# tenstack/batch-scheduler

Hardware: AMD Instinct MI355X
Metric: pod x node fit evals/sec (higher is better)
Workload: dtype int64; 1 GPU; cfg3/tail: 10000 pods / 2000 groups / 5000 nodes, 5 int64 lanes (cpu, mem, eph, pods, gpu), seed 20260921; stages=prefilter+filter+tally+ready, parallelism=single GPU

## Files before the change

### batch-scheduler_amd/csrc/bs_fast.hpp

```cpp
#pragma once

#include "bs_kernels.hpp"
#include "bs_filter_t.hpp"

#ifdef BS_NT_TABLES
#define BS_TBL_STORE(p, v) __builtin_nontemporal_store((v), (p))
#else
#define BS_TBL_STORE(p, v) (*(p) = (v))
#endif
namespace bs {

template <bool INL = false>
__device__ __forceinline__ void arm_tally(const GroupsDev& gr, const BatchDev& b, const BatchParams& prm, uint32_t i, uint32_t nthreads);

__device__ __forceinline__ const uint8_t* range_glocal(const BatchDev& b) { return reinterpret_cast<const uint8_t*>(b.pod_ranges); }
__device__ __forceinline__ const uint32_t* range_start(const BatchDev& b, uint32_t G) { return b.pod_ranges + (G + 3u) / 4u; }
__device__ __forceinline__ const uint32_t* range_lfirst(const BatchDev& b, uint32_t G, uint32_t pod_blocks) { return range_start(b, G) + pod_blocks + 1u; }
__device__ __forceinline__ bool range_local_on(const BatchDev& b, const BatchParams& prm) {
  return b.pod_ranges && prm.do_tally && prm.do_ready && !prm.filter_deny;
}

#if BS_EMIT_MAIN
__global__ void k_pods_prep(unsigned long long* tables, uint32_t ntab, uint32_t* gstat, uint32_t ngstat, uint32_t* kcount, uint32_t* gcount, uint32_t G) {
  const uint32_t t = blockIdx.x * blockDim.x + threadIdx.x, nt = gridDim.x * blockDim.x;
// ... 166 lines not shown
      al[j] = nd.alloc[(size_t)j * nd.stride + n];
      rq[j] = nd.req[(size_t)j * nd.stride + n];
    }
  }
  const bool fit = valid && ((fw >> (n & 31u)) & 1u) && !(fl & BS_NODE_TAINT_ERR);
  const uint32_t pres = fit ? (ap & rp) : 0u;
  BS_STAMP(1, 1);
  if (threadIdx.x < BS_MAX_SCALARS) s_kp[threadIdx.x] = BS_INF;
  unsigned long long incl[BS_MAX_LANES];
  const int w = wave_id();
#pragma unroll
  for (uint32_t j = 0; j < BS_MAX_LANES; ++j) {
    if (j < L) {
      const bool live = fit && (j < 4 || (pres & (1u << (j - 4)))) && !(j == BS_LANE_EPH && !prm.eph_gate);
      const unsigned long long left = live ? (unsigned long long)wsub(scale_f32(al[j], d.pct), rq[j]) : 0ull;
      incl[j] = wave_incl_scan_add_u64(left);
      if (lane_id() == 63) s_wtot[j][w] = incl[j];
    }
  }
  __syncthreads();
#pragma unroll
  for (uint32_t j = 0; j < BS_MAX_LANES; ++j) {
    if (j < L) {
      unsigned long long off = 0, tot = 0;
#pragma unroll
      for (int i = 0; i < 4; ++i) {
        const unsigned long long x = s_wtot[j][i];
        if (i < w) off += x;
        tot += x;
      }
      incl[j] += off;
      if (valid) BS_TBL_STORE(&T[(size_t)k * LP + j], (int64_t)incl[j]);
      if (threadIdx.x == 0) b.chunk_tot[(size_t)chunk * 16 + j] = tot;
    } else if (j < LP && valid) {
      BS_TBL_STORE(&T[(size_t)k * LP + j], (int64_t)INT64_MAX);
    }
  }
  {
    const uint32_t grp = k >> 6;
    const bool grp_valid = (chunk * kTblChunk + (threadIdx.x & ~63u)) < nd.m;
    constexpr int64_t kSafe = (int64_t)1 << 62;
#pragma unroll
    for (uint32_t j = 0; j < BS_MAX_LANES; ++j) {
      if (j < L) {
        const int64_t x = (int64_t)incl[j];
        const long long mx = wave_max_i64_lane63(valid ? x : INT64_MIN);
        const bool risky = __ballot(valid && (x >= kSafe || x <= -kSafe)) != 0ull;
        if (lane_id() == 63 && grp_valid) b.gmax[(size_t)grp * LP + j] = risky ? INT64_MAX : mx;
      }
    }
  }
#pragma unroll
  for (uint32_t s = 0; s < BS_MAX_SCALARS; ++s) {
    if (s < S) {
      const unsigned long long mk = __ballot(valid && (pres & (1u << s)));
      if (mk && lane_id() == 0) atomicMin(&s_kp[s], chunk * kTblChunk + (uint32_t)(threadIdx.x & ~63u) + (uint32_t)(__ffsll((long long)mk) - 1));
    }
  }
  __syncthreads();
  if (threadIdx.x < 16) b.chunk_kp[(size_t)chunk * 16 + threadIdx.x] = threadIdx.x < BS_MAX_SCALARS ? s_kp[threadIdx.x] : BS_INF;
}

struct LeaderPre { Res mr; bool have_mr; int64_t min_member, status_scheduled, matched; };
template <bool PUB, typename T>
__device__ __forceinline__ void st_pub(T* p, T v) {
  if constexpr (PUB) __hip_atomic_store(p, v, __ATOMIC_RELAXED, __HIP_MEMORY_SCOPE_AGENT);
  else *p = v;
}
#ifndef BS_HOME_WT
#define BS_HOME_WT 0
#endif
template <typename T>
__device__ __forceinline__ void st_home(T* p, T v) {
#if BS_HOME_WT
  __hip_atomic_store(p, v, __ATOMIC_RELAXED, __HIP_MEMORY_SCOPE_SYSTEM);
#else
  *p = v;
#endif
}
__device__ __forceinline__ uint32_t ld_agent(const uint32_t* p) { return __hip_atomic_load(p, __ATOMIC_RELAXED, __HIP_MEMORY_SCOPE_AGENT); }
__device__ __forceinline__ unsigned long long ld_agent64(const void* p) {
  return __hip_atomic_load(reinterpret_cast<const unsigned long long*>(p), __ATOMIC_RELAXED, __HIP_MEMORY_SCOPE_AGENT);
}
template <int TS>
__device__ __forceinline__ void leader_pre_load(const GroupsDev& gr, int32_t leader, Shape<TS> sh, LeaderPre& o) {
  const uint32_t l = leader >= 0 ? (uint32_t)leader : 0u;
#pragma unroll
  for (uint32_t j = 0; j < BS_MAX_LANES; ++j) o.mr.v[j] = j < sh.L() ? gr.minres[(size_t)j * gr.g + l] : 0;
  o.mr.present = gr.mrpres[l];
  o.have_mr = (gr.flags[l] & BS_GROUP_HAS_MINRES) != 0;
  o.min_member = (int64_t)gr.min_member[l];
  o.status_scheduled = (int64_t)gr.status_scheduled[l];
  o.matched = (int64_t)gr.matched[l];
}
template <int TS>
__device__ __forceinline__ void pre_allocated_from(const LeaderPre& lp, Shape<TS> sh, uint32_t gate, Res& out) {
  res_zero(out, sh);
  const int64_t mm = lp.min_member;
  const int64_t not_finished = lp.matched != 0 ? mm - lp.matched : mm - lp.status_scheduled;
  if (not_finished > 0 && lp.have_mr) {
    Res times;
#pragma unroll
    for (uint32_t j = 0; j < BS_MAX_LANES; ++j)
      if (j < sh.L()) times.v[j] = wmul(lp.mr.v[j], not_finished);
    times.present = lp.mr.present;
    res_add(out, times, sh, gate);
  }
  if (out.v[BS_LANE_PODS] == 0) out.v[BS_LANE_PODS] = mm + 1;
}
template <int TS>
__device__ __forceinline__ uint32_t filter_slot_values(const Res& cur_in, const LeaderPre& lp, Shape<TS> sh, uint32_t gate, int64_t (&R)[4], int64_t (&M)[4]) {
  Res ms, cur = cur_in;
  res_zero(ms, sh);
  res_add(ms, lp.mr, sh, gate);
  res_add(cur, ms, sh, gate);
  uint32_t ff = 0;
#pragma unroll
  for (uint32_t s = 0; s < BS_MAX_SCALARS; ++s) {
    if (s < sh.S()) {
      if ((cur.present & (1u << s)) && cur.v[4 + s] != 0) ff |= 1u;
      if ((ms.present & (1u << s)) && ms.v[4 + s] != 0) ff |= 2u;
    }
  }
#pragma unroll
  for (int j = 0; j < 4; ++j) { R[j] = cur.v[j]; M[j] = ms.v[j]; }
  return ff;
}
template <int TS, bool PUB = false>
__device__ __forceinline__ void filter_slot_from(const BatchDev& b, const BatchParams& prm, const Res& cur_in, const LeaderPre& lp, Shape<TS> sh, uint32_t gate,
                                                 uint32_t slot, bool zero_feas = true) {
  if (!lp.have_mr) return;
  int64_t R[4], M[4];
  const uint32_t ff = filter_slot_values(cur_in, lp, sh, gate, R, M);
  if (zero_feas) st_pub<PUB>(&b.fu_feas[slot], 0u);
  int64_t* dst2 = b.uparams + (size_t)slot * 8;
#pragma unroll
  for (int j = 0; j < 4; ++j) { st_pub<PUB>(&dst2[j], R[j]); st_pub<PUB>(&dst2[4 + j], M[j]); }
  st_pub<PUB>(&b.uflags[slot], ff | ((uint32_t)BS_FL_EVALUATED << 8) | (prm.stamp << 16));
}
template <int TS>
__device__ __forceinline__ uint32_t class_scan_query(const Res& cur, const LeaderPre& lp0, Shape<TS> sh, uint32_t gate, Res& q) {
  pre_allocated_from(lp0, sh, gate, q);
  res_add(q, cur, sh, gate);
  uint32_t absok = 0;
#pragma unroll
  for (uint32_t s2 = 0; s2 < BS_MAX_SCALARS; ++s2) {
    if (s2 < sh.S()) {
      const bool pres = q.present & (1u << s2);
      if (!pres || q.v[4 + s2] == 0) absok |= 1u << s2;
      if (!pres) q.v[4 + s2] = INT64_MIN;
    }
  }
  return q.present | (absok << 16);
}

template <int TS, bool PUB = false, bool SLOTS = true, bool INL = false>
__device__ __forceinline__ void fast_query_thread(const PodsDev& pods, const GroupsDev& gr, const BatchDev& b, const BatchParams& prm, uint32_t i,
                                                  uint32_t nthreads, uint32_t end = BS_INF, uint32_t t = BS_INF) {
  const Shape<TS> sh(prm.S);
  const bool valid = i < pods.p && i < end;
  const uint32_t gate = prm.eph_gate;
  const uint32_t ii = valid ? i : 0u;
  const int32_t leader0 = b.leader_epoch[0];
  const uint8_t panic0 = b.panic_epoch[0];
  const uint32_t K = prm.run_filter ? (prm.k_host ? prm.k_host : *b.kclass) : 0u;
  const int32_t gi = pods.p ? pods.group[ii] : BS_POD_NOT_GROUPED;
  const uint8_t pfl = pods.p ? pods.flags[ii] : (uint8_t)0;
  const uint64_t own = pods.p ? pods.owner[ii] : 0ull;
  const uint32_t pc = pods.p ? b.pclass[ii] : 0u;
  const uint32_t pp = pods.p ? b.ppair[ii] : BS_INF;
  Res cur;
  if (pods.p) pod_require(pods, ii, sh, gate, cur); else res_zero(cur, sh);
  arm_tally<INL>(gr, b, prm, t == BS_INF ? i : t, nthreads);
  if (i < 8 && prm.collect_stats) b.stats[i] = 0;
  const bool grouped = valid && gi >= 0 && (uint32_t)gi < gr.g;
  const uint32_t g = grouped ? (uint32_t)gi : 0u;
// ... 152 lines not shown
template <int TS>
__global__ __launch_bounds__(kTblChunk) void k_fast_query_tables(PodsDev pods, GroupsDev gr, NodesDev nd, BatchDev b, BatchDev bt, BatchParams prm,
                                                                 const TableDesc* forced, uint32_t nchunks, uint32_t query_blocks) {
  BS_STAMP(1, 0);
  if (blockIdx.x < query_blocks) fast_query_thread<TS>(pods, gr, b, prm, blockIdx.x * kTblChunk + threadIdx.x, query_blocks * kTblChunk);
  else if (blockIdx.x < query_blocks + nchunks) tables_local_fast<TS>(nd, bt, prm, forced, blockIdx.x - query_blocks);
  else node_words_block<TS>(gr, nd, b, prm, blockIdx.x - query_blocks - nchunks);
  BS_STAMP(1, 7);
}

template <int NL>
__device__ __forceinline__ unsigned long long rows_cover(unsigned long long m, const int64_t (&a)[BS_MAX_LANES], const int64_t (&r)[BS_MAX_LANES]) {
  asm volatile("s_mov_b64 exec, %[m]\n\tv_cmpx_ge_i64 vcc, %[a0], %[r0]\n\tv_cmpx_ge_i64 vcc, %[a1], %[r1]\n\tv_cmpx_ge_i64 vcc, %[a2], %[r2]\n\t"
               "v_cmpx_ge_i64 vcc, %[a3], %[r3]\n\ts_mov_b64 %[m], exec\n\ts_mov_b64 exec, -1"
               : [m] "+s"(m)
               : [a0] "v"(a[0]), [r0] "v"(r[0]), [a1] "v"(a[1]), [r1] "v"(r[1]), [a2] "v"(a[2]), [r2] "v"(r[2]), [a3] "v"(a[3]), [r3] "v"(r[3])
               : "vcc");
#pragma unroll
  for (int j = 4; j < NL; ++j)
    asm volatile("s_mov_b64 exec, %[m]\n\tv_cmpx_ge_i64 vcc, %[a], %[r]\n\ts_mov_b64 %[m], exec\n\ts_mov_b64 exec, -1" : [m] "+s"(m) : [a] "v"(a[j]), [r] "v"(r[j]) : "vcc");
  return m;
}
#ifndef BS_SCAN_BALLOT
#define BS_SCAN_BALLOT 1
#endif
constexpr uint32_t kSpinBound = 1u << 18;
__device__ __forceinline__ void test_chaos_delay() {
#ifdef BS_TEST_CHAOS
  uint32_t h = (blockIdx.x + 1u) * 2654435761u ^ (uint32_t)wall_clock64() * 40503u;
  h ^= h >> 15; h *= 2246822519u; h ^= h >> 13;
  for (uint32_t s = 0; s < (h & 15u); ++s) __builtin_amdgcn_s_sleep(127);
#endif
}
constexpr uint32_t kStepSlotsMax = 256;
__device__ __forceinline__ bool step_wait(const uint32_t* word, uint32_t base, uint32_t need, int32_t* h_err) {
  uint32_t spins = 0;
  while ((uint32_t)(ld_agent(word) - base) < need) {
    __builtin_amdgcn_s_sleep(1);
    if (++spins > kSpinBound) { if (h_err) __hip_atomic_store(h_err, 1, __ATOMIC_RELAXED, __HIP_MEMORY_SCOPE_SYSTEM); return false; }
  }
  return true;
}
constexpr uint32_t kScanRecChunks = 64;
constexpr uint32_t kFeasRecGroups = 32;
#ifndef BS_GATHER_DIRECT
#define BS_GATHER_DIRECT 8
#endif
constexpr uint32_t kGatherDirectBlocks = BS_GATHER_DIRECT;
constexpr uint32_t kRecStride = 32;
constexpr uint32_t kTkSlots = 32, kTkTab = 48, kTkP1 = 64, kTkDone = 64 + 16 * 16, kTkWays = 16, kTkWords = 64 + 2 * 16 * 16;
__device__ __forceinline__ void spread_add(uint32_t* words, uint32_t who) {
  (void)__hip_atomic_fetch_add(&words[16u * (who % kTkWays)], 1u, __ATOMIC_RELAXED, __HIP_MEMORY_SCOPE_AGENT);
}
__device__ __forceinline__ bool spread_wait(const uint32_t* words, uint32_t base, uint32_t need, int32_t* h_err) {
  uint32_t spins = 0;
  for (;;) {
    uint32_t v = lane_id() < (int)kTkWays ? ld_agent(&words[16u * (uint32_t)lane_id()]) : 0u;
#pragma unroll
    for (int o = 1; o < (int)kTkWays; o <<= 1) v += (uint32_t)__shfl_xor((int)v, o);
    v = (uint32_t)__builtin_amdgcn_readfirstlane((int)v);
    if ((uint32_t)(v - base) >= need) return true;
    __builtin_amdgcn_s_sleep(4);
    if (++spins > kSpinBound) { if (h_err && lane_id() == 0) __hip_atomic_store(h_err, 1, __ATOMIC_RELAXED, __HIP_MEMORY_SCOPE_SYSTEM); return false; }
  }
}
template <int TS, bool REGS = false>
__device__ __forceinline__ void table_scan_block(const NodesDev& nd, const BatchDev& b, const BatchParams& prm, const TableDesc* forced, uint32_t chunk, uint32_t nchunks,
                                                 uint32_t share, uint32_t nshares, uint32_t pod_blocks, uint32_t tk_pods0, uint32_t tk_tab0, const GroupsDev& gr,
                                                 const int64_t* ckeys, const uint32_t* cpres, uint32_t kcap, bool direct = false, uint32_t forced_cls = 0) {
  __shared__ unsigned long long s_wtot[BS_MAX_LANES][4];
  __shared__ uint32_t s_kp[BS_MAX_SCALARS];
  __shared__ unsigned long long s_off[BS_MAX_LANES];
  __shared__ uint32_t s_kpg[BS_MAX_SCALARS];
  __shared__ int64_t s_req[kStepSlotsMax][BS_MAX_LANES];
  __shared__ uint32_t s_qf[kStepSlotsMax];
  __shared__ uint32_t s_first[kStepSlotsMax];
  BS_STAMP(2, 0);
  const Shape<TS> sh(prm.S);
  const uint32_t L = sh.L(), S = sh.S(), LP = prm.LP;
  const uint32_t k = chunk * kTblChunk + threadIdx.x;
  const bool in_range = REGS ? k < nd.n : k < nd.m;
  const uint32_t n = REGS ? (in_range ? k : 0u) : (in_range ? nd.kmap[k] : 0u);
  const TableDesc d = REGS ? TableDesc{forced_cls, 0.7f} : *forced;
  const uint32_t fw = nd.fit[(size_t)d.cls * nd.fit_words + (n >> 5)];
  const uint8_t fl = nd.flags[n];
  const bool valid = in_range && (!REGS || !(fl & BS_NODE_SKIP_MASK));
  const uint32_t ap = nd.apres[n], rp = nd.rpres[n];
  int64_t al[BS_MAX_LANES], rq[BS_MAX_LANES];
#pragma unroll
  for (uint32_t j = 0; j < BS_MAX_LANES; ++j) {
    if (j < L) {
      al[j] = nd.alloc[(size_t)j * nd.stride + n];
      rq[j] = nd.req[(size_t)j * nd.stride + n];
    }
  }
  const uint32_t K = prm.k_host ? prm.k_host : *b.kclass;
  const uint32_t per = (K + nshares - 1u) / nshares, s_lo = share * per, s_hi = min(K, s_lo + per);
  Res raw;
  int32_t leader0 = -1;
  uint8_t panic0 = 0;
  LeaderPre lp0{};
  if constexpr (REGS) {
    const uint32_t cc = s_lo + threadIdx.x < s_hi ? s_lo + threadIdx.x : 0u;
#pragma unroll
    for (uint32_t j = 0; j < BS_MAX_LANES; ++j)
      if (j < L) raw.v[j] = ckeys[(size_t)j * kcap + cc];
    raw.present = cpres[cc];
    leader0 = b.leader_epoch[0];
    panic0 = b.panic_epoch[0];
    if (gr.g) leader_pre_load(gr, leader0, sh, lp0);
  }
  const bool fit = valid && ((fw >> (n & 31u)) & 1u) && !(fl & BS_NODE_TAINT_ERR);
  const uint32_t pres = fit ? (ap & rp) : 0u;
  if (threadIdx.x < BS_MAX_SCALARS) s_kp[threadIdx.x] = BS_INF;
  for (uint32_t t = threadIdx.x; t < kStepSlotsMax; t += kTblChunk) s_first[t] = BS_INF;
  unsigned long long incl[BS_MAX_LANES];
  const int w = wave_id();
#pragma unroll
  for (uint32_t j = 0; j < BS_MAX_LANES; ++j) {
    incl[j] = 0;
    if (j < L) {
      const bool live = fit && (j < 4 || (pres & (1u << (j - 4)))) && !(j == BS_LANE_EPH && !prm.eph_gate);
      const unsigned long long left = live ? (unsigned long long)wsub(scale_f32(al[j], d.pct), rq[j]) : 0ull;
      incl[j] = wave_incl_scan_add_u64(left);
      if (lane_id() == 63) s_wtot[j][w] = incl[j];
    }
  }
  __syncthreads();
#pragma unroll
  for (uint32_t s2 = 0; s2 < BS_MAX_SCALARS; ++s2) {
    if (s2 < S) {
      const unsigned long long mk = __ballot(valid && (pres & (1u << s2)));
      if (mk && lane_id() == 0) atomicMin(&s_kp[s2], chunk * kTblChunk + (uint32_t)(threadIdx.x & ~63u) + (uint32_t)(__ffsll((long long)mk) - 1));
    }
  }
#pragma unroll
  for (uint32_t j = 0; j < BS_MAX_LANES; ++j) {
    if (j < L) {
      unsigned long long off = 0, tot = 0;
#pragma unroll
      for (int i = 0; i < 4; ++i) {
        const unsigned long long x = s_wtot[j][i];
        if (i < w) off += x;
        tot += x;
      }
      incl[j] += off;
      if (threadIdx.x == 0 && share == 0) {
        if constexpr (REGS) {
          const unsigned long long tag = (unsigned long long)prm.seq_inv << 32;
          st_pub<true>(&b.chunk_rec[(size_t)chunk * kRecStride + 2u * j], tag | (uint32_t)tot);
          st_pub<true>(&b.chunk_rec[(size_t)chunk * kRecStride + 2u * j + 1u], tag | (uint32_t)(tot >> 32));
        } else {
          st_pub<true>(&b.chunk_tot[(size_t)chunk * 16 + j], tot);
        }
      }
    }
  }
  __syncthreads();
  __shared__ uint32_t s_ok;
  if constexpr (REGS) {
    if (share == 0 && threadIdx.x < S) st_pub<true>(&b.chunk_rec[(size_t)chunk * kRecStride + 16u + threadIdx.x], ((unsigned long long)prm.seq_inv << 32) | s_kp[threadIdx.x]);
    BS_STAMP(2, 1);
  } else {
    if (share == 0 && threadIdx.x < 16) st_pub<true>(&b.chunk_kp[(size_t)chunk * 16 + threadIdx.x], threadIdx.x < BS_MAX_SCALARS ? s_kp[threadIdx.x] : BS_INF);
    asm volatile("s_waitcnt vmcnt(0)" ::: "memory");
    __syncthreads();
    BS_STAMP(2, 1);
    if (threadIdx.x == 0 && share == 0) (void)__hip_atomic_fetch_add(&b.ticket[kTkTab], 1u, __ATOMIC_RELAXED, __HIP_MEMORY_SCOPE_AGENT);
  }
  if constexpr (REGS) {
    const uint32_t t = s_lo + threadIdx.x;
    if (t < s_hi) {
      uint32_t qf = 0x80000000u;
      Res q;
      res_zero(q, sh);
      if (leader0 >= 0 && !panic0) {
        Res cur;
        res_zero(cur, sh);
        res_add(cur, raw, sh, prm.eph_gate);
        qf = class_scan_query(cur, lp0, sh, prm.eph_gate, q);
      }
      s_qf[threadIdx.x] = qf;
#pragma unroll
      for (uint32_t j = 0; j < BS_MAX_LANES; ++j)
        if (j < L) s_req[threadIdx.x][j] = q.v[j];
    }
  }
  if constexpr (!REGS) {
    if (threadIdx.x == 0) s_ok = (step_wait(&b.ticket[kTkTab], tk_tab0, nchunks, b.h_err) && step_wait(&b.ticket[kTkSlots], tk_pods0, pod_blocks, b.h_err)) ? 1u : 0u;
    __syncthreads();
    BS_STAMP(2, 2);
    if (!s_ok) return;
  }
  {
    const uint32_t ch = (uint32_t)lane_id();
    unsigned long long cv[BS_MAX_LANES];
    uint32_t ckp[BS_MAX_SCALARS];
    if constexpr (REGS) {
      if (w == 0) {
        const uint32_t tagw = prm.seq_inv;
        const unsigned long long* rec = b.chunk_rec + (size_t)(ch < nchunks ? ch : 0u) * kRecStride;
        bool ok = false;
        for (uint32_t spins = 0;; ++spins) {
          unsigned long long lo[BS_MAX_LANES], hi[BS_MAX_LANES], kw[BS_MAX_SCALARS];
#pragma unroll
          for (uint32_t j = 0; j < BS_MAX_LANES; ++j)
            if (j < L) { lo[j] = ld_agent64(&rec[2u * j]); hi[j] = ld_agent64(&rec[2u * j + 1u]); }
#pragma unroll
          for (uint32_t s2 = 0; s2 < BS_MAX_SCALARS; ++s2)
            if (s2 < S) kw[s2] = ld_agent64(&rec[16u + s2]);
          bool mine_ok = true;
#pragma unroll
          for (uint32_t j = 0; j < BS_MAX_LANES; ++j) {
            cv[j] = 0ull;
            if (j < L) {
              mine_ok = mine_ok && (uint32_t)(lo[j] >> 32) == tagw && (uint32_t)(hi[j] >> 32) == tagw;
              cv[j] = (hi[j] << 32) | (uint32_t)lo[j];
            }
          }
#pragma unroll
          for (uint32_t s2 = 0; s2 < BS_MAX_SCALARS; ++s2) {
            ckp[s2] = BS_INF;
            if (s2 < S) { mine_ok = mine_ok && (uint32_t)(kw[s2] >> 32) == tagw; ckp[s2] = (uint32_t)kw[s2]; }
          }
          if (__ballot(!(mine_ok || ch >= nchunks)) == 0ull) { ok = true; break; }
          if (spins > kSpinBound) { if (b.h_err && ch == 0) __hip_atomic_store(b.h_err, 1, __ATOMIC_RELAXED, __HIP_MEMORY_SCOPE_SYSTEM); break; }
          __builtin_amdgcn_s_sleep(2);
        }
        if (ch >= nchunks) {
#pragma unroll
          for (uint32_t j = 0; j < BS_MAX_LANES; ++j) cv[j] = 0ull;
#pragma unroll
          for (uint32_t s2 = 0; s2 < BS_MAX_SCALARS; ++s2) ckp[s2] = BS_INF;
        }
        if (ch == 0) s_ok = ok ? 1u : 0u;
      }
      BS_STAMP(2, 2);
    } else if (w == 0) {
#pragma unroll
      for (uint32_t j = 0; j < BS_MAX_LANES; ++j) cv[j] = (j < L && ch < nchunks) ? ld_agent64(&b.chunk_tot[(size_t)ch * 16 + j]) : 0ull;
#pragma unroll
      for (uint32_t s2 = 0; s2 < BS_MAX_SCALARS; ++s2) ckp[s2] = (s2 < S && ch < nchunks) ? ld_agent(&b.chunk_kp[(size_t)ch * 16 + s2]) : BS_INF;
    }
    const uint32_t t = s_lo + threadIdx.x;
    uint32_t stp = 0, qf = 0x80000000u;
    int32_t tab = -1;
    unsigned long long rv[BS_MAX_LANES];
    if (!REGS && t < s_hi) {
      stp = ld_agent(&b.qstamp_s[t]);
      tab = (int32_t)ld_agent(reinterpret_cast<const uint32_t*>(&b.qtab_s[t]));
      qf = ld_agent(&b.qflags_s[t]);
#pragma unroll
      for (uint32_t j = 0; j < BS_MAX_LANES; ++j) rv[j] = j < L ? ld_agent64(&b.qreq_s[(size_t)t * LP + j]) : 0ull;
// ... 28 lines not shown
    if (!s_ok) return;
  }
  int64_t fin[BS_MAX_LANES];
  uint32_t keyrow = 0;
#pragma unroll
  for (uint32_t j = 0; j < BS_MAX_LANES; ++j) {
    fin[j] = 0;
    if (j < L) fin[j] = (int64_t)(incl[j] + s_off[j]);
  }
#pragma unroll
  for (uint32_t s2 = 0; s2 < BS_MAX_SCALARS; ++s2)
    if (s2 < S && k >= s_kpg[s2]) keyrow |= 1u << s2;
  BS_STAMP(2, 3);
  const uint32_t nmine = s_hi > s_lo ? s_hi - s_lo : 0u;
  const uint32_t smask = S ? ((1u << S) - 1u) : 0u;
  const uint32_t row0 = chunk * kTblChunk + ((uint32_t)w << 6);
  for (uint32_t t0 = 0; t0 < nmine; t0 += 4u) {
    uint32_t qf[4];
    int64_t r[4][BS_MAX_LANES];
#pragma unroll
    for (uint32_t u = 0; u < 4; ++u) {
      const uint32_t t = min(t0 + u, nmine - 1u);
      qf[u] = t0 + u < nmine ? s_qf[t] : 0x80000000u;
#pragma unroll
      for (uint32_t j = 0; j < BS_MAX_LANES; ++j) r[u][j] = j < L ? s_req[t][j] : 0;
    }
#pragma unroll
    for (uint32_t u = 0; u < 4; ++u) {
      const uint32_t nab = ~(qf[u] >> 16) & smask;
      unsigned long long m = (qf[u] & 0x80000000u) ? 0ull : __ballot(valid && (nab & ~keyrow) == 0u);
      static_assert(TS >= 0 && TS <= 4, "k_fast_step_a is instantiated for 0..4 scalar lanes (run_fast: step_a_possible)");
#if BS_SCAN_BALLOT
#pragma unroll
      for (uint32_t j = 0; j < 4u + (uint32_t)TS; ++j) m &= __ballot(fin[j] >= r[u][j]);
#else
      m = rows_cover<4 + TS>(m, fin, r[u]);
#endif
      if (m && lane_id() == 0) atomicMin(&s_first[t0 + u], row0 + (uint32_t)(__ffsll((long long)m) - 1));
    }
  }
  __syncthreads();
  BS_STAMP(2, 4);
  if constexpr (REGS) {
    if (direct) {
      for (uint32_t t = threadIdx.x; t < nmine; t += kTblChunk)
        st_pub<true>(&b.scan_rec[(size_t)chunk * kStepSlotsMax + s_lo + t], ((unsigned long long)prm.seq_inv << 32) | s_first[t]);
    } else {
      for (uint32_t t = threadIdx.x; t < nmine; t += kTblChunk)
        if (s_first[t] != BS_INF) atomicMin(&b.first_row64[s_lo + t], ((unsigned long long)prm.seq_inv << 32) | s_first[t]);
    }
    BS_STAMP(2, 7);
    return;
  }
  for (uint32_t t = threadIdx.x; t < nmine; t += kTblChunk) {
    if (s_first[t] == BS_INF) continue;
    atomicMin(&b.first_row[s_lo + t], s_first[t]);
  }
  BS_STAMP(2, 7);
}

__device__ __forceinline__ void step_filter_split(uint32_t K, uint32_t W, uint32_t target_waves, uint32_t& tiles, uint32_t& bpw, uint32_t& nchunk) {
  tiles = (2u * K + 63u) / 64u;
  uint32_t nsplit = max(1u, target_waves / max(tiles, 1u));
  nsplit = min(nsplit, max((W + 1u) / 2u, 1u));
  bpw = max(2u, (((W + nsplit - 1u) / nsplit + 1u) / 2u) * 2u);
  nchunk = (W + bpw - 1u) / bpw;
  if ((nchunk + 3u) / 4u > kFeasRecGroups) {
    bpw = ((W + 4u * kFeasRecGroups - 1u) / (4u * kFeasRecGroups) + 1u) / 2u * 2u;
    nchunk = (W + bpw - 1u) / bpw;
  }
}
template <int TS>
__device__ __forceinline__ void step_filter_block(const GroupsDev& gr, const NodesDev& nd, const BatchDev& b, const BatchParams& prm, const int64_t* ckeys,
                                                  const uint32_t* cpres, uint32_t kcap, uint32_t target_waves, uint32_t ustride, uint32_t bx, uint32_t nblocks,
                                                  bool direct, uint32_t tk_slots0, uint32_t slot_producers) {
  __shared__ uint32_t s_cnt[4][64];
  BS_STAMP_AT(4, 0, bx);
  const Shape<TS> sh(prm.S);
  const uint32_t gate = prm.eph_gate, K = prm.k_host ? prm.k_host : (uint32_t)__builtin_amdgcn_readfirstlane((int)*b.kclass), U = 2u * K;
  const uint32_t W = (nd.n + 63u) / 64u;
  if (!U || !W) return;
  uint32_t tiles, bpw, nchunk;
  step_filter_split(K, W, target_waves, tiles, bpw, nchunk);
  const uint32_t groups = (nchunk + 3u) / 4u;
  const int32_t leader0 = b.leader_epoch[0];
  LeaderPre lp0{}, lp1{};
  const bool two = prm.sop_leader0 >= 0 && prm.sop_leader0 != leader0;
  if (gr.g) {
    leader_pre_load(gr, leader0, sh, lp0);
    if (two) leader_pre_load(gr, prm.sop_leader0, sh, lp1); else lp1 = lp0;
  }
  bool waited = false;
  for (uint32_t bi = bx; bi < tiles * groups; bi += nblocks) {
    const uint32_t tile = bi % tiles, group = bi / tiles, chunk = group * 4u + (uint32_t)wave_id();
    const uint32_t src = tile * 64u + (uint32_t)lane_id();
    const bool second = src >= K;
    const uint32_t c = src < U ? (second ? src - K : src) : 0u;
    uint32_t cnt = 0;
    if (chunk < nchunk) {
      Res raw;
#pragma unroll
      for (uint32_t j = 0; j < BS_MAX_LANES; ++j)
        if (j < sh.L()) raw.v[j] = ckeys[(size_t)j * kcap + c];
      raw.present = cpres[c];
      Res cur;
      res_zero(cur, sh);
      res_add(cur, raw, sh, gate);
      LeaderPre lp = lp0;
      if (second) lp = lp1;
      const bool on = src < U && (second ? prm.sop_leader0 >= 0 : leader0 >= 0) && lp.have_mr;
      int64_t R[4], M[4];
      const uint32_t ff = filter_slot_values(cur, lp, sh, gate, R, M);
      filter_item<2, 4, true, true>(nd, b, U, ustride, tile, chunk * bpw, min(W, chunk * bpw + bpw), 0u,
                                    on ? (ff | ((uint32_t)BS_FL_EVALUATED << 8)) : ((uint32_t)BS_FL_NOT_RUN << 8), R, M, &cnt);
    }
    s_cnt[wave_id()][lane_id()] = cnt;
    BS_STAMP_AT(4, 1, bx);
    if (direct && b.h_rows) asm volatile("s_waitcnt vmcnt(0)" ::: "memory");
    __syncthreads();
    BS_STAMP_AT(4, 2, bx);
    if (wave_id() == 0 && src < U) {
      const uint32_t sum = s_cnt[0][lane_id()] + s_cnt[1][lane_id()] + s_cnt[2][lane_id()] + s_cnt[3][lane_id()];
      if (direct) {
        st_pub<true>(&b.feas_rec[(size_t)group * (2u * kStepSlotsMax) + src], ((unsigned long long)prm.seq_inv << 32) | sum);
      } else {
        if (!waited) { (void)step_wait(&b.ticket[kTkSlots], tk_slots0, slot_producers, b.h_err); waited = true; }
        if (sum) atomicAdd(&b.fu_feas[src], sum);
      }
    }
    __syncthreads();
  }
  BS_STAMP_AT(4, 7, bx);
}

template <int TS>
__device__ __forceinline__ void class_slots_block(const GroupsDev& gr, const BatchDev& b, const BatchParams& prm, const int64_t* ckeys, const uint32_t* cpres,
                                                  uint32_t kcap, uint32_t blk, bool zero_feas) {
  const Shape<TS> sh(prm.S);
#ifdef BS_TEST_OLD_ZERO
  zero_feas = true;
#endif
  const uint32_t gate = prm.eph_gate, K = prm.k_host ? prm.k_host : *b.kclass;
  const uint32_t c = blk * kTblChunk + threadIdx.x;
  Res raw;
  const uint32_t cc = c < K ? c : 0u;
#pragma unroll
  for (uint32_t j = 0; j < BS_MAX_LANES; ++j)
    if (j < sh.L()) raw.v[j] = ckeys[(size_t)j * kcap + cc];
  raw.present = cpres[cc];
  const int32_t leader0 = b.leader_epoch[0];
  const uint8_t panic0 = b.panic_epoch[0];
  LeaderPre lp0{}, lp1{};
  const bool two = prm.run_filter && prm.sop_leader0 >= 0 && prm.sop_leader0 != leader0;
  if (gr.g) {
    leader_pre_load(gr, leader0, sh, lp0);
    if (two) leader_pre_load(gr, prm.sop_leader0, sh, lp1); else lp1 = lp0;
  }
  if (c < K) {
    Res cur;
    res_zero(cur, sh);
    res_add(cur, raw, sh, gate);
    if (leader0 >= 0 && !panic0) {
      Res q;
      const uint32_t qfw = class_scan_query(cur, lp0, sh, gate, q);
      int64_t* dst = b.qreq_s + (size_t)c * prm.LP;
#pragma unroll
      for (uint32_t j = 0; j < BS_MAX_LANES; ++j)
        if (j < prm.LP) st_pub<true>(&dst[j], j < sh.L() ? q.v[j] : (int64_t)INT64_MIN);
      st_pub<true>(&b.qflags_s[c], qfw);
      st_pub<true>(&b.qtab_s[c], (int32_t)0);
      st_pub<true>(&b.first_row[c], BS_INF);
      st_pub<true>(&b.qstamp_s[c], prm.stamp);
    }
    if (prm.run_filter) {
      if (leader0 >= 0) filter_slot_from<TS, true>(b, prm, cur, lp0, sh, gate, c, zero_feas);
      if (prm.sop_leader0 >= 0) filter_slot_from<TS, true>(b, prm, cur, lp1, sh, gate, c + K, zero_feas);
    }
  }
  BS_STAMP(1, 4);
  asm volatile("s_waitcnt vmcnt(0)" ::: "memory");
  __syncthreads();
  BS_STAMP(1, 5);
  if (threadIdx.x == 0) (void)__hip_atomic_fetch_add(&b.ticket[kTkSlots], 1u, __ATOMIC_RELAXED, __HIP_MEMORY_SCOPE_AGENT);
}


template <bool INL>
__device__ __forceinline__ void arm_tally(const GroupsDev& gr, const BatchDev& b, const BatchParams& prm, uint32_t i, uint32_t nthreads) {
  if (i == 0) __hip_atomic_store(&b.ticket[1], 0u, __ATOMIC_RELAXED, __HIP_MEMORY_SCOPE_AGENT);
  for (uint32_t g = i; g < gr.g; g += nthreads) {
    if (INL && range_local_on(b, prm) && range_glocal(b)[g]) continue;
    st_pub<INL>(&b.admit[g], 0u);
    if (prm.do_ready) {
      st_pub<INL>(&b.admit64[g], 0ull);
      if (b.gcount[g] == 0u) {
        const uint8_t rd = gr.matched[g] >= (uint32_t)(gr.min_member[g] - gr.status_scheduled[g]) ? 1 : 0;
        b.ready[g] = rd;
        if (prm.host_tag) { st_home(&b.h_admit[g], 0u); st_home(&b.h_ready[g], rd); }
      }
    }
  }
}

template <bool WT = false>
__device__ __forceinline__ void final_tail(const BatchDev& b, const BatchParams& prm, uint32_t nblocks) {
  __shared__ uint32_t s_last;
  if (!prm.host_tag) return;
  if constexpr (WT && BS_HOME_WT) asm volatile("s_waitcnt vmcnt(0)" ::: "memory");
  else __builtin_amdgcn_fence(__ATOMIC_RELEASE, "");
  __syncthreads();
  if (threadIdx.x == 0) s_last = __hip_atomic_fetch_add(&b.ticket[0], 1u, __ATOMIC_RELAXED, __HIP_MEMORY_SCOPE_AGENT) == nblocks - 1 ? 1u : 0u;
  __syncthreads();
  if (!s_last) return;
// ... 548 lines not shown
```

### batch-scheduler_amd/csrc/bs_kernels.hpp

```cpp
#pragma once

#include "bs_common.hpp"
#include "bs_nodew_layout.hpp"

namespace bs {

struct NodesDev {
  uint32_t n, stride;
  const int64_t* alloc;
  const int64_t* req;
  const uint32_t* apres;
  const uint32_t* rpres;
  const uint8_t* flags;
  const uint32_t* fit;
  uint32_t fit_words, n_classes;
  const uint32_t* kmap;
  uint32_t m;
  const int64_t* left4;
  const int64_t* lglob;
};

struct GroupsDev {
  uint32_t g;
  const uint32_t* min_member;
// ... 1486 lines not shown
__global__ void k_filter_params(PodsDev pods, GroupsDev gr, BatchDev b, BatchParams prm) {
  const uint32_t i = blockIdx.x * blockDim.x + threadIdx.x;
  if (i >= pods.p) return;
  filter_params_for<-1>(pods, gr, b, prm, i, b.pf_code[i], b.pf_leader[i], i, true, true);
}
#endif

template <int TS>
__global__ void k_fparams_early(PodsDev pods, GroupsDev gr, BatchDev b, BatchParams prm) {
  const uint32_t i = blockIdx.x * blockDim.x + threadIdx.x;
  if (i >= pods.p) return;
  const uint8_t pf = (b.stage[i] & ST_OWNED) ? b.tcode[i] : (uint8_t)BS_PF_NOT_OWNED;
  const bool after = i >= b.nepochs[1];
  const int32_t leader = after ? b.leader_epoch[0] : prm.sop_leader0;
  const uint32_t slot = prm.use_classes ? b.pclass[i] + (after ? 0u : *b.kclass) : i;
  filter_params_for<TS>(pods, gr, b, prm, i, pf, leader, slot, true, true);
}

#define BS_OPT_0(x) ""
#define BS_OPT_1(x) x
#define BS_OPT(flag, x) BS_OPT_##flag(x)
template <int MASK>
__device__ __forceinline__ void filter_pod2(uint32_t pp, const int64_t (&R)[4], unsigned long long ok0, unsigned long long ok1,
                                            const int64_t (&l0)[4], const int64_t (&l1)[4], uint32_t& vlo0, uint32_t& vhi0,
                                            uint32_t& vlo1, uint32_t& vhi1);
#define BS_DEF_FILTER_POD2(MASK, f0, f1, f2, f3)                                                                          \
  template <>                                                                                                             \
  __device__ __forceinline__ void filter_pod2<MASK>(uint32_t pp, const int64_t (&R)[4], unsigned long long ok0,          \
                                                    unsigned long long ok1, const int64_t (&l0)[4], const int64_t (&l1)[4], \
                                                    uint32_t& vlo0, uint32_t& vhi0, uint32_t& vlo1, uint32_t& vhi1) {       \
    asm volatile("s_mov_b32 m0, %[pp]\n\t"                                                                                \
                 "s_mov_b64 exec, %[ok0]\n\t"                                                                             \
                 BS_OPT(f0, "v_cmpx_le_i64 vcc, %[R0], %[a0]\n\t") BS_OPT(f1, "v_cmpx_le_i64 vcc, %[R1], %[a1]\n\t")       \
                 BS_OPT(f2, "v_cmpx_le_i64 vcc, %[R2], %[a2]\n\t") BS_OPT(f3, "v_cmpx_le_i64 vcc, %[R3], %[a3]\n\t")       \
                 "s_nop 3\n\t"                                                                                            \
                 "v_writelane_b32 %[vlo0], exec_lo, m0\n\t"                                                               \
                 "v_writelane_b32 %[vhi0], exec_hi, m0\n\t"                                                               \
                 "s_mov_b64 exec, %[ok1]\n\t"                                                                             \
                 BS_OPT(f0, "v_cmpx_le_i64 vcc, %[R0], %[b0]\n\t") BS_OPT(f1, "v_cmpx_le_i64 vcc, %[R1], %[b1]\n\t")       \
                 BS_OPT(f2, "v_cmpx_le_i64 vcc, %[R2], %[b2]\n\t") BS_OPT(f3, "v_cmpx_le_i64 vcc, %[R3], %[b3]\n\t")       \
                 "s_nop 3\n\t"                                                                                            \
                 "v_writelane_b32 %[vlo1], exec_lo, m0\n\t"                                                               \
                 "v_writelane_b32 %[vhi1], exec_hi, m0\n\t"                                                               \
                 "s_mov_b64 exec, -1"                                                                                     \
                 : [vlo0] "+v"(vlo0), [vhi0] "+v"(vhi0), [vlo1] "+v"(vlo1), [vhi1] "+v"(vhi1)                             \
                 : [pp] "s"(pp), [ok0] "s"(ok0), [ok1] "s"(ok1), [R0] "v"(R[0]), [R1] "v"(R[1]), [R2] "v"(R[2]),          \
                   [R3] "v"(R[3]), [a0] "v"(l0[0]), [a1] "v"(l0[1]), [a2] "v"(l0[2]), [a3] "v"(l0[3]), [b0] "v"(l1[0]),   \
                   [b1] "v"(l1[1]), [b2] "v"(l1[2]), [b3] "v"(l1[3])                                                      \
                 : "vcc");                                                                                                \
  }
BS_DEF_FILTER_POD2(1, 1, 0, 0, 0)
BS_DEF_FILTER_POD2(2, 0, 1, 0, 0)
BS_DEF_FILTER_POD2(3, 1, 1, 0, 0)
BS_DEF_FILTER_POD2(4, 0, 0, 1, 0)
BS_DEF_FILTER_POD2(5, 1, 0, 1, 0)
BS_DEF_FILTER_POD2(6, 0, 1, 1, 0)
BS_DEF_FILTER_POD2(7, 1, 1, 1, 0)
BS_DEF_FILTER_POD2(8, 0, 0, 0, 1)
BS_DEF_FILTER_POD2(9, 1, 0, 0, 1)
BS_DEF_FILTER_POD2(10, 0, 1, 0, 1)
BS_DEF_FILTER_POD2(11, 1, 1, 0, 1)
BS_DEF_FILTER_POD2(12, 0, 0, 1, 1)
BS_DEF_FILTER_POD2(13, 1, 0, 1, 1)
BS_DEF_FILTER_POD2(14, 0, 1, 1, 1)
BS_DEF_FILTER_POD2(15, 1, 1, 1, 1)

template <int MASK, int PU = 4>
__device__ __forceinline__ void filter_pod_loop(uint32_t np, const int64_t (*sR)[4], const unsigned long long (&okmask)[2],
                                                const int64_t (&l)[2][4], uint32_t (&vlo)[2], uint32_t (&vhi)[2]) {
  for (uint32_t pp = 0; pp < np; pp += PU) {
    int64_t R[PU][4];
#pragma unroll
    for (int u = 0; u < PU; ++u) {
      const uint32_t pu = min(pp + (uint32_t)u, np - 1);
#pragma unroll
      for (int j = 0; j < 4; ++j) R[u][j] = ((MASK >> j) & 1) ? sR[pu][j] : 0;
    }
#pragma unroll
    for (int u = 0; u < PU; ++u)
      filter_pod2<MASK>(min(pp + (uint32_t)u, np - 1), R[u], okmask[0], okmask[1], l[0], l[1], vlo[0], vhi[0], vlo[1], vhi[1]);
  }
}

template <int NB, int PU = 4, bool DB = true, bool REGS = false>
__device__ __forceinline__ void filter_item(const NodesDev& nd, const BatchDev& b, uint32_t U, uint32_t ustride, uint32_t ptile,
                                            uint32_t w0, uint32_t w1, uint32_t stamp = 0, uint32_t ff_in = 0, const int64_t* R_in = nullptr,
                                            const int64_t* M_in = nullptr, uint32_t* cnt_out = nullptr) {
  static_assert(NB == 2, "the inner statement handles two node blocks");
  typedef const __attribute__((address_space(4))) uint32_t* cflag_t;
  const int lane = lane_id();
  const uint32_t p0 = ptile * 64u;
  const uint32_t np = min(64u, U - p0);

  const bool mine = (uint32_t)lane < np;
  const uint32_t src = p0 + (uint32_t)lane;
  uint32_t myff = (uint32_t)BS_FL_NOT_RUN << 8;
  int64_t M[4] = {0, 0, 0, 0}, myR[4] = {0, 0, 0, 0};
  if constexpr (REGS) {
    if (mine) {
      myff = ff_in;
#pragma unroll
      for (int j = 0; j < 4; ++j) { myR[j] = R_in[j]; M[j] = M_in[j]; }
    }
  } else if (mine) {
    myff = b.uflags[src];
    const int64_t* rs = b.uparams + (size_t)src * 8;
#pragma unroll
    for (int j = 0; j < 4; ++j) { myR[j] = rs[j]; M[j] = rs[4 + j]; }
  }
  int64_t gl[8];
#pragma unroll
  for (int j = 0; j < 8; ++j) gl[j] = nd.lglob[j];
  int64_t l[NB][4], ln[NB][4];
  uint8_t nfl[NB], nfln[NB];
  auto load_blocks = [&](uint32_t w, int64_t (&dst)[NB][4], uint8_t (&fl)[NB]) {
#pragma unroll
    for (int nb = 0; nb < NB; ++nb) {
      const uint32_t n = (w + nb) * 64u + (uint32_t)lane;
      const bool nvalid = (w + nb) < w1 && n < nd.n;
      fl[nb] = 0xFF;
#pragma unroll
      for (int j = 0; j < 4; ++j) dst[nb][j] = INT64_MIN;
      if (nvalid) {
#pragma unroll
        for (int j = 0; j < 4; ++j) dst[nb][j] = nd.left4[(size_t)j * nd.stride + n];
        fl[nb] = nd.flags[n];
      }
    }
  };
  load_blocks(w0, l, nfl);
  if (!REGS && stamp) myff = (myff >> 16) == stamp ? (myff & 0xFFFFu) : ((uint32_t)BS_FL_NOT_RUN << 8);
  const uint32_t myfl = myff >> 8;
  const bool ev = myfl == BS_FL_EVALUATED;
  if (!ev) {
#pragma unroll
    for (int j = 0; j < 4; ++j) M[j] = 0;
  }
  __shared__ int64_t s_R[4][64][4];
  __builtin_amdgcn_wave_barrier();
  uint32_t lane_mask = 0;
  bool tile_allfail = false;
  {
#pragma unroll
    for (int j = 0; j < 4; ++j) s_R[wave_id()][lane][j] = myR[j];
    __builtin_amdgcn_wave_barrier();
    const bool c2pod = ev && !(myff & 1u);
    const unsigned long long c2mask = __ballot(c2pod);
#pragma unroll
    for (int j = 0; j < 4; ++j) {
      if (__ballot(c2pod && !(gl[j] >= myR[j]))) lane_mask |= 1u << j;
      if (c2mask && !__ballot(c2pod && gl[4 + j] >= myR[j])) tile_allfail = true;
    }
  }
  const unsigned long long evmask = __ballot(ev);
  if (!evmask) return;
  bool uniformM = true;
  int64_t M0[4] = {0, 0, 0, 0};
  uint32_t lb0 = 0;
  if (evmask) {
    const int first = __ffsll((long long)evmask) - 1;
    bool same = true;
#pragma unroll
    for (int j = 0; j < 4; ++j) {
      M0[j] = __shfl(M[j], first);
      same = same && (M[j] == M0[j]);
    }
    lb0 = (uint32_t)__shfl((int)(myff & 2u), first);
    same = same && ((myff & 2u) == lb0);
    uniformM = __ballot(ev && !same) == 0;
  }

  crow_t FP = as_const_rows(b.uparams);
  cflag_t FF = (cflag_t)(uintptr_t)b.uflags;
  uint32_t cnt = 0;
  for (uint32_t w = w0; w < w1; w += NB) {
    if constexpr (DB) {
      if (w + NB < w1) load_blocks(w + NB, ln, nfln);
    }
    unsigned long long okmask[NB], in_range[NB], nlf[NB];
    uint32_t vlo[NB], vhi[NB];
#pragma unroll
    for (int nb = 0; nb < NB; ++nb) {
      const bool nvalid = nfl[nb] != 0xFF;
      const bool node_ok = nvalid && !(nfl[nb] & (BS_NODE_NIL | BS_NODE_NO_NODE));
      in_range[nb] = __ballot(nvalid);
      okmask[nb] = __ballot(node_ok);
      unsigned long long lf = 0;
      if (!lb0) lf = __ballot(l[nb][0] >= M0[0]) & __ballot(l[nb][1] >= M0[1]) & __ballot(l[nb][2] >= M0[2]) & __ballot(l[nb][3] >= M0[3]);
      nlf[nb] = okmask[nb] & ~lf;
      vlo[nb] = 0;
      vhi[nb] = 0;
    }
    if (uniformM) {
      const int64_t (*sR)[4] = s_R[wave_id()];
      if (tile_allfail) {
      } else {
        switch (lane_mask) {
          case 0:
#pragma unroll
            for (int nb = 0; nb < NB; ++nb) { vlo[nb] = (uint32_t)okmask[nb]; vhi[nb] = (uint32_t)(okmask[nb] >> 32); }
            break;
          case 1: filter_pod_loop<1, PU>(np, sR, okmask, l, vlo, vhi); break;
          case 2: filter_pod_loop<2, PU>(np, sR, okmask, l, vlo, vhi); break;
          case 3: filter_pod_loop<3, PU>(np, sR, okmask, l, vlo, vhi); break;
          case 4: filter_pod_loop<4, PU>(np, sR, okmask, l, vlo, vhi); break;
          case 5: filter_pod_loop<5, PU>(np, sR, okmask, l, vlo, vhi); break;
          case 6: filter_pod_loop<6, PU>(np, sR, okmask, l, vlo, vhi); break;
          case 7: filter_pod_loop<7, PU>(np, sR, okmask, l, vlo, vhi); break;
          case 8: filter_pod_loop<8, PU>(np, sR, okmask, l, vlo, vhi); break;
          case 9: filter_pod_loop<9, PU>(np, sR, okmask, l, vlo, vhi); break;
          case 10: filter_pod_loop<10, PU>(np, sR, okmask, l, vlo, vhi); break;
          case 11: filter_pod_loop<11, PU>(np, sR, okmask, l, vlo, vhi); break;
          case 12: filter_pod_loop<12, PU>(np, sR, okmask, l, vlo, vhi); break;
// ... 281 lines not shown
```

Baseline: 3763 billion evals/s.

## Issue leader and node-block loads early to overlap latency in filter and table scan

Splits the leader precompute load into an issue phase and a use phase, using a zero VGPR offset, lane-distributed minres loads and broadcasts so the loads are vector loads issued early. The filter step now issues the class-key, node-block and leader loads for each item up front, with sched barriers, and feeds them into filter_item through a new PRE path. It also peeks the slot ticket early so the blocking wait can be skipped when producers are already done. The goal is to hide global memory latency behind other work, at the cost of more live registers and an explicit full waitcnt at the end of each iteration.

Result: slower. 3690 billion evals/s (-2.0%).

```diff
diff --git a/batch-scheduler_amd/csrc/bs_fast.hpp b/batch-scheduler_amd/csrc/bs_fast.hpp
--- a/batch-scheduler_amd/csrc/bs_fast.hpp
+++ b/batch-scheduler_amd/csrc/bs_fast.hpp
@@ -272,16 +272,61 @@
 __device__ __forceinline__ unsigned long long ld_agent64(const void* p) {
   return __hip_atomic_load(reinterpret_cast<const unsigned long long*>(p), __ATOMIC_RELAXED, __HIP_MEMORY_SCOPE_AGENT);
 }
+struct LeaderRaw { int64_t mr[BS_MAX_LANES]; uint32_t mrpres, min_member, status_scheduled, matched; uint8_t flags; };
+__device__ __forceinline__ uint32_t lane_zero() {
+  uint32_t z;
+  asm volatile("v_mov_b32 %0, 0" : "=v"(z));
+  return z;
+}
+template <int TS>
+__device__ __forceinline__ void leader_pre_issue(const GroupsDev& gr, int32_t leader, Shape<TS> sh, uint32_t z, LeaderRaw& r, bool counts = true) {
+  const uint32_t l = (leader >= 0 ? (uint32_t)leader : 0u) + z;
+#pragma unroll
+  for (uint32_t j = 0; j < BS_MAX_LANES; ++j) r.mr[j] = j < sh.L() ? gr.minres[(size_t)j * gr.g + l] : 0;
+  r.mrpres = gr.mrpres[l];
+  r.flags = gr.flags[l];
+  if (counts) {
+    r.min_member = gr.min_member[l];
+    r.status_scheduled = gr.status_scheduled[l];
+    r.matched = gr.matched[l];
+  }
+}
+__device__ __forceinline__ void leader_pre_use(const LeaderRaw& r, LeaderPre& o) {
+#pragma unroll
+  for (uint32_t j = 0; j < BS_MAX_LANES; ++j) o.mr.v[j] = r.mr[j];
+  o.mr.present = r.mrpres;
+  o.have_mr = (r.flags & BS_GROUP_HAS_MINRES) != 0;
+  o.min_member = (int64_t)r.min_member;
+  o.status_scheduled = (int64_t)r.status_scheduled;
+  o.matched = (int64_t)r.matched;
+}
+struct LeaderRawLanes { int64_t mrl; uint32_t mrpres, min_member, status_scheduled, matched, flags; };
+template <int TS>
+__device__ __forceinline__ void leader_pre_issue(const GroupsDev& gr, int32_t leader, Shape<TS> sh, uint32_t z, LeaderRawLanes& r) {
+  const uint32_t l0 = leader >= 0 ? (uint32_t)leader : 0u, l = l0 + z;
+  r.mrl = gr.minres[(size_t)min((uint32_t)lane_id(), sh.L() - 1u) * gr.g + l0];
+  r.mrpres = gr.mrpres[l];
+  r.flags = gr.flags[l];
+  r.min_member = gr.min_member[l];
+  r.status_scheduled = gr.status_scheduled[l];
+  r.matched = gr.matched[l];
+}
+template <int TS>
+__device__ __forceinline__ void leader_pre_use(LeaderRawLanes r, Shape<TS> sh, LeaderPre& o) {
+  asm volatile("" : "+v"(r.mrl), "+v"(r.mrpres), "+v"(r.flags), "+v"(r.min_member), "+v"(r.status_scheduled), "+v"(r.matched));
+#pragma unroll
+  for (uint32_t j = 0; j < BS_MAX_LANES; ++j) o.mr.v[j] = j < sh.L() ? (int64_t)bcast64((uint64_t)r.mrl, (int)j) : 0;
+  o.mr.present = r.mrpres;
+  o.have_mr = (r.flags & BS_GROUP_HAS_MINRES) != 0;
+  o.min_member = (int64_t)r.min_member;
+  o.status_scheduled = (int64_t)r.status_scheduled;
+  o.matched = (int64_t)r.matched;
+}
 template <int TS>
 __device__ __forceinline__ void leader_pre_load(const GroupsDev& gr, int32_t leader, Shape<TS> sh, LeaderPre& o) {
-  const uint32_t l = leader >= 0 ? (uint32_t)leader : 0u;
-#pragma unroll
-  for (uint32_t j = 0; j < BS_MAX_LANES; ++j) o.mr.v[j] = j < sh.L() ? gr.minres[(size_t)j * gr.g + l] : 0;
-  o.mr.present = gr.mrpres[l];
-  o.have_mr = (gr.flags[l] & BS_GROUP_HAS_MINRES) != 0;
-  o.min_member = (int64_t)gr.min_member[l];
-  o.status_scheduled = (int64_t)gr.status_scheduled[l];
-  o.matched = (int64_t)gr.matched[l];
+  LeaderRaw r;
+  leader_pre_issue(gr, leader, sh, 0u, r);
+  leader_pre_use(r, o);
 }
 template <int TS>
 __device__ __forceinline__ void pre_allocated_from(const LeaderPre& lp, Shape<TS> sh, uint32_t gate, Res& out) {
@@ -600,6 +645,12 @@
   const bool in_range = REGS ? k < nd.n : k < nd.m;
   const uint32_t n = REGS ? (in_range ? k : 0u) : (in_range ? nd.kmap[k] : 0u);
   const TableDesc d = REGS ? TableDesc{forced_cls, 0.7f} : *forced;
+  int32_t leader0 = -1;
+  uint8_t panic0 = 0;
+  if constexpr (REGS) {
+    leader0 = b.leader_epoch[0];
+    panic0 = b.panic_epoch[0];
+  }
   const uint32_t fw = nd.fit[(size_t)d.cls * nd.fit_words + (n >> 5)];
   const uint8_t fl = nd.flags[n];
   const bool valid = in_range && (!REGS || !(fl & BS_NODE_SKIP_MASK));
@@ -615,18 +666,16 @@
   const uint32_t K = prm.k_host ? prm.k_host : *b.kclass;
   const uint32_t per = (K + nshares - 1u) / nshares, s_lo = share * per, s_hi = min(K, s_lo + per);
   Res raw;
-  int32_t leader0 = -1;
-  uint8_t panic0 = 0;
-  LeaderPre lp0{};
+  LeaderRawLanes lr0{};
   if constexpr (REGS) {
     const uint32_t cc = s_lo + threadIdx.x < s_hi ? s_lo + threadIdx.x : 0u;
 #pragma unroll
     for (uint32_t j = 0; j < BS_MAX_LANES; ++j)
       if (j < L) raw.v[j] = ckeys[(size_t)j * kcap + cc];
     raw.present = cpres[cc];
-    leader0 = b.leader_epoch[0];
-    panic0 = b.panic_epoch[0];
-    if (gr.g) leader_pre_load(gr, leader0, sh, lp0);
+    __builtin_amdgcn_sched_barrier(0);
+    if (gr.g) leader_pre_issue(gr, leader0, sh, lane_zero(), lr0);
+    __builtin_amdgcn_sched_barrier(0);
   }
   const bool fit = valid && ((fw >> (n & 31u)) & 1u) && !(fl & BS_NODE_TAINT_ERR);
   const uint32_t pres = fit ? (ap & rp) : 0u;
@@ -687,6 +736,9 @@
     if (threadIdx.x == 0 && share == 0) (void)__hip_atomic_fetch_add(&b.ticket[kTkTab], 1u, __ATOMIC_RELAXED, __HIP_MEMORY_SCOPE_AGENT);
   }
   if constexpr (REGS) {
+    __builtin_amdgcn_sched_barrier(0);
+    LeaderPre lp0;
+    leader_pre_use(lr0, sh, lp0);
     const uint32_t t = s_lo + threadIdx.x;
     if (t < s_hi) {
       uint32_t qf = 0x80000000u;
@@ -881,37 +933,54 @@
   if (!U || !W) return;
   uint32_t tiles, bpw, nchunk;
   step_filter_split(K, W, target_waves, tiles, bpw, nchunk);
-  const uint32_t groups = (nchunk + 3u) / 4u;
-  const int32_t leader0 = b.leader_epoch[0];
-  LeaderPre lp0{}, lp1{};
-  const bool two = prm.sop_leader0 >= 0 && prm.sop_leader0 != leader0;
-  if (gr.g) {
-    leader_pre_load(gr, leader0, sh, lp0);
-    if (two) leader_pre_load(gr, prm.sop_leader0, sh, lp1); else lp1 = lp0;
-  }
+  const uint32_t groups = (nchunk + 3u) / 4u, items = tiles * groups;
+  int32_t leader0 = -1;
+  const uint32_t wv = (uint32_t)__builtin_amdgcn_readfirstlane(wave_id());
+  auto item_issue = [&](uint32_t bi, Res& raw, FilterPre& pre) {
+    const uint32_t src = (bi % tiles) * 64u + (uint32_t)lane_id(), chunk = (bi / tiles) * 4u + wv;
+    const uint32_t c = src < U ? (src >= K ? src - K : src) : 0u;
+#pragma unroll
+    for (uint32_t j = 0; j < BS_MAX_LANES; ++j)
+      if (j < sh.L()) raw.v[j] = ckeys[(size_t)j * kcap + c];
+    raw.present = cpres[c];
+    filter_pre_load(nd, chunk * bpw, min(W, chunk * bpw + bpw), pre);
+  };
+  auto leader_issue = [&](uint32_t bi, int32_t l0, LeaderRaw& lr) {
+    const bool second = (bi % tiles) * 64u + (uint32_t)lane_id() >= K;
+    if (gr.g) leader_pre_issue(gr, second && prm.sop_leader0 >= 0 ? prm.sop_leader0 : l0, sh, 0u, lr, false);
+  };
   bool waited = false;
-  for (uint32_t bi = bx; bi < tiles * groups; bi += nblocks) {
-    const uint32_t tile = bi % tiles, group = bi / tiles, chunk = group * 4u + (uint32_t)wave_id();
+  for (uint32_t bi = bx; bi < items; bi += nblocks) {
+    const uint32_t tile = bi % tiles, group = bi / tiles, chunk = group * 4u + wv;
     const uint32_t src = tile * 64u + (uint32_t)lane_id();
     const bool second = src >= K;
-    const uint32_t c = src < U ? (second ? src - K : src) : 0u;
+    Res raw;
+    FilterPre pre;
+    LeaderRaw lr{};
+    if (bi == bx) leader0 = b.leader_epoch[lane_zero()];
+    item_issue(bi, raw, pre);
+    __builtin_amdgcn_sched_barrier(0);
+    int32_t l0 = leader0;
+    asm volatile("" : "+v"(l0));
+    leader_issue(bi, l0, lr);
+    __builtin_amdgcn_sched_barrier(0);
+    uint32_t early = tk_slots0;
+    if (!direct && !waited && wave_id() == 0) {
+      early = ld_agent(&b.ticket[kTkSlots]);
+      __builtin_amdgcn_sched_barrier(0);
+    }
     uint32_t cnt = 0;
     if (chunk < nchunk) {
-      Res raw;
-#pragma unroll
-      for (uint32_t j = 0; j < BS_MAX_LANES; ++j)
-        if (j < sh.L()) raw.v[j] = ckeys[(size_t)j * kcap + c];
-      raw.present = cpres[c];
       Res cur;
       res_zero(cur, sh);
       res_add(cur, raw, sh, gate);
-      LeaderPre lp = lp0;
-      if (second) lp = lp1;
-      const bool on = src < U && (second ? prm.sop_leader0 >= 0 : leader0 >= 0) && lp.have_mr;
+      LeaderPre lp;
+      leader_pre_use(lr, lp);
+      const bool on = src < U && (second ? prm.sop_leader0 >= 0 : l0 >= 0) && lp.have_mr;
       int64_t R[4], M[4];
       const uint32_t ff = filter_slot_values(cur, lp, sh, gate, R, M);
-      filter_item<2, 4, true, true>(nd, b, U, ustride, tile, chunk * bpw, min(W, chunk * bpw + bpw), 0u,
-                                    on ? (ff | ((uint32_t)BS_FL_EVALUATED << 8)) : ((uint32_t)BS_FL_NOT_RUN << 8), R, M, &cnt);
+      filter_item<2, 4, true, true, true>(nd, b, U, ustride, tile, chunk * bpw, min(W, chunk * bpw + bpw), 0u,
+                                          on ? (ff | ((uint32_t)BS_FL_EVALUATED << 8)) : ((uint32_t)BS_FL_NOT_RUN << 8), R, M, &cnt, &pre);
     }
     s_cnt[wave_id()][lane_id()] = cnt;
     BS_STAMP_AT(4, 1, bx);
@@ -923,11 +992,15 @@
       if (direct) {
         st_pub<true>(&b.feas_rec[(size_t)group * (2u * kStepSlotsMax) + src], ((unsigned long long)prm.seq_inv << 32) | sum);
       } else {
-        if (!waited) { (void)step_wait(&b.ticket[kTkSlots], tk_slots0, slot_producers, b.h_err); waited = true; }
+        if (!waited) {
+          if ((uint32_t)(early - tk_slots0) < slot_producers) (void)step_wait(&b.ticket[kTkSlots], tk_slots0, slot_producers, b.h_err);
+          waited = true;
+        }
         if (sum) atomicAdd(&b.fu_feas[src], sum);
       }
     }
     __syncthreads();
+    __builtin_amdgcn_s_waitcnt(0x0F70);
   }
   BS_STAMP_AT(4, 7, bx);
 }
diff --git a/batch-scheduler_amd/csrc/bs_kernels.hpp b/batch-scheduler_amd/csrc/bs_kernels.hpp
--- a/batch-scheduler_amd/csrc/bs_kernels.hpp
+++ b/batch-scheduler_amd/csrc/bs_kernels.hpp
@@ -1592,10 +1592,27 @@
   }
 }
 
-template <int NB, int PU = 4, bool DB = true, bool REGS = false>
+struct FilterPre { int64_t gll; int64_t l[2][4]; uint8_t fl[2]; };
+__device__ __forceinline__ void filter_pre_load(const NodesDev& nd, uint32_t w0, uint32_t w1, FilterPre& o) {
+  o.gll = nd.lglob[lane_id() & 7];
+#pragma unroll
+  for (uint32_t nb = 0; nb < 2; ++nb) {
+    const uint32_t n = (w0 + nb) * 64u + (uint32_t)lane_id();
+    const bool nvalid = (w0 + nb) < w1 && n < nd.n;
+    o.fl[nb] = 0xFF;
+#pragma unroll
+    for (int j = 0; j < 4; ++j) o.l[nb][j] = INT64_MIN;
+    if (nvalid) {
+#pragma unroll
+      for (int j = 0; j < 4; ++j) o.l[nb][j] = nd.left4[(size_t)j * nd.stride + n];
+      o.fl[nb] = nd.flags[n];
+    }
+  }
+}
+template <int NB, int PU = 4, bool DB = true, bool REGS = false, bool PRE = false>
 __device__ __forceinline__ void filter_item(const NodesDev& nd, const BatchDev& b, uint32_t U, uint32_t ustride, uint32_t ptile,
                                             uint32_t w0, uint32_t w1, uint32_t stamp = 0, uint32_t ff_in = 0, const int64_t* R_in = nullptr,
-                                            const int64_t* M_in = nullptr, uint32_t* cnt_out = nullptr) {
+                                            const int64_t* M_in = nullptr, uint32_t* cnt_out = nullptr, const FilterPre* pre = nullptr) {
   static_assert(NB == 2, "the inner statement handles two node blocks");
   typedef const __attribute__((address_space(4))) uint32_t* cflag_t;
   const int lane = lane_id();
@@ -1620,7 +1637,7 @@
   }
   int64_t gl[8];
 #pragma unroll
-  for (int j = 0; j < 8; ++j) gl[j] = nd.lglob[j];
+  for (int j = 0; j < 8; ++j) gl[j] = PRE ? (int64_t)bcast64((uint64_t)pre->gll, j) : nd.lglob[j];
   int64_t l[NB][4], ln[NB][4];
   uint8_t nfl[NB], nfln[NB];
   auto load_blocks = [&](uint32_t w, int64_t (&dst)[NB][4], uint8_t (&fl)[NB]) {
@@ -1638,7 +1655,16 @@
       }
     }
   };
-  load_blocks(w0, l, nfl);
+  if constexpr (PRE) {
+#pragma unroll
+    for (int nb = 0; nb < NB; ++nb) {
+      nfl[nb] = pre->fl[nb];
+#pragma unroll
+      for (int j = 0; j < 4; ++j) l[nb][j] = pre->l[nb][j];
+    }
+  } else {
+    load_blocks(w0, l, nfl);
+  }
   if (!REGS && stamp) myff = (myff >> 16) == stamp ? (myff & 0xFFFFu) : ((uint32_t)BS_FL_NOT_RUN << 8);
   const uint32_t myfl = myff >> 8;
   const bool ev = myfl == BS_FL_EVALUATED;
```
